# ofsoundof/NTIRE2022_ESR

Measured on AMD Instinct MI355X. Metric: images/sec (256x256->1024x1024 x4), higher is better.
Workload: dtype f32

## Files before the change

include/esr_hip.h:

```cpp
#ifndef ESR_HIP_H
#define ESR_HIP_H

#include <stddef.h>
#include <stdint.h>

#ifdef __cplusplus
extern "C" {
#endif

#define ESR_ABI_VERSION 12

typedef enum esr_status {
    ESR_OK = 0,
    ESR_ERR_BAD_ARG = -1,
    ESR_ERR_UNSUPPORTED = -2,
    ESR_ERR_LAUNCH = -3,
    ESR_ERR_TOO_SMALL = -4
} esr_status;

typedef enum esr_act { ESR_ACT_NONE = 0, ESR_ACT_LRELU = 1, ESR_ACT_RELU = 2, ESR_ACT_GELU = 3 } esr_act;

typedef enum esr_res { ESR_RES_NONE = 0, ESR_RES_PRE_ACT = 1, ESR_RES_POST_ACT = 2, ESR_RES_GATE = 3 } esr_res;

typedef enum esr_compute { ESR_COMPUTE_F32 = 0, ESR_COMPUTE_BF16 = 1, ESR_COMPUTE_F16 = 2 } esr_compute;
// ... 63 lines not shown
int    esr_pack_tail_s16(const float* w, const float* bias, int nseg, int seg_c, int mid_c, int cout, int compute, void* out, size_t out_bytes);
int    esr_conv_tail_supported(const esr_conv_desc* d);
int    esr_pack_conv_f32(const float* w_oihw, const float* bias, int cin, int cout, int ksize,
                         const int32_t* cin_map, int cin_phys, void* out, size_t out_bytes);
int    esr_unpack_conv_f32(const void* packed, size_t bytes, int cin, int cout, int ksize,
                           const int32_t* cin_map, int cin_phys, float* w_oihw, float* bias);

size_t esr_packed_conv_s16_bytes(int cin_phys, int cout, int ksize);
int    esr_pack_conv_s16(const float* w_oihw, const float* bias, int cin, int cout, int ksize, const int32_t* cin_map,
                         int cin_phys, int compute, void* out, size_t out_bytes);
int    esr_unpack_conv_s16(const void* packed, size_t bytes, int cin, int cout, int ksize, const int32_t* cin_map,
                           int cin_phys, int compute, float* w_oihw, float* bias);

size_t esr_packed_post_s16_bytes(int cin, int cout);
int    esr_pack_post_s16(const float* w_oi, const float* bias, int cin, int cout, int compute, void* out, size_t out_bytes);
int    esr_conv_post_supported(const esr_conv_desc* d);

size_t esr_packed_wino_bytes(int cin_phys, int cout);
int    esr_pack_wino_f32(const float* w_oihw, const float* bias, int cin, int cout, const int32_t* cin_map, int cin_phys,
                         void* out, size_t out_bytes);
int    esr_unpack_wino_f32(const void* packed, size_t bytes, int cin, int cout, const int32_t* cin_map, int cin_phys,
                           float* u_oc16, float* bias);
int    esr_wino_supported(const esr_conv_desc* d);

int esr_conv2d_f32(const esr_conv_desc* d, void* hip_stream);
int esr_conv_block_waves(const esr_conv_desc* d);

#define ESR_ESA_FP 16

size_t esr_packed_dense_bytes(int cin_p, int cout_p, int ksize);
int    esr_pack_dense_f32(const float* w_oihw, const float* bias, int cin, int cout, int ksize,
                          int cin_p, int cout_p, void* out, size_t out_bytes);

typedef struct esr_esa_post {
    int32_t cout;
    int32_t act;
    float   slope;
    int32_t res_mode;
    esr_view res;
    esr_view out;
} esr_esa_post;
int    esr_esa_apply_post_supported(int c, int cout0, int cout1);
size_t esr_packed_apply_post_bytes(int cin, int cout0, int cout1, int storage);
int    esr_pack_apply_post(const float* w0, const float* b0, const float* w1, const float* b1, int cin, int cout0, int cout1,
                           int storage, void* out, size_t out_bytes);

// ... 213 lines not shown
```

ntire2022_esr_amd/_lib.py:

```python
import ctypes
import os

_HERE = os.path.dirname(os.path.abspath(__file__))
SO_PATH = os.environ.get("ESR_HIP_LIB") or os.path.join(_HERE, "libesr_hip.so")

ESR_OK = 0
STATUS = {0: "ESR_OK", -1: "ESR_ERR_BAD_ARG", -2: "ESR_ERR_UNSUPPORTED", -3: "ESR_ERR_LAUNCH", -4: "ESR_ERR_TOO_SMALL"}

ACT_NONE, ACT_LRELU, ACT_RELU, ACT_GELU = 0, 1, 2, 3
RES_NONE, RES_PRE_ACT, RES_POST_ACT, RES_GATE = 0, 1, 2, 3
NHWC, NCHW_IN, NCHW_SHUFFLE4 = 0, 1, 2
BLOCKED_IN, BLOCKED_OUT1, BLOCKED_OUT0, BLOCKED_RES = 1, 2, 4, 8
HILO_IN, HILO_RES, HILO_OUT = 1, 2, 4
OP_CONV, OP_CONV3X3S2, OP_MAXPOOL7S3, OP_ESA_APPLY, OP_DWCONV, OP_BSCONV, OP_PACK_INPUT, OP_ESA_LOWRES, OP_CONV_CHAIN = 0, 1, 2, 3, 4, 5, 6, 7, 8
OP_MAXPOOL7S7 = 9
OP_DISTILL_STEP = 10
OP_RESBLOCK_HEAD = 11
OP_REFINE_CASCADE = 12
OP_DWCONV7 = 13
OP_CX_BLOCK = 14
OP_DWPW_PAIR = 15
OP_ESA_UNSHUFFLE = 16
OP_PA_GATE = 17
OP_PA_TAIL = 18
# ... 88 lines not shown
class ChainDesc(ctypes.Structure):
    _fields_ = [
        ("n", ctypes.c_int32), ("h", ctypes.c_int32), ("w", ctypes.c_int32), ("n_layers", ctypes.c_int32),
        ("cin", ctypes.c_int32), ("cmid", ctypes.c_int32), ("cout", ctypes.c_int32),
        ("act", ctypes.c_int32), ("slope", ctypes.c_float), ("res_mode", ctypes.c_int32),
        ("storage", ctypes.c_int32), ("compute", ctypes.c_int32),
        ("inp", View), ("wpacked", ctypes.c_void_p * CHAIN_MAX_LAYERS),
        ("post_wpacked", ctypes.c_void_p), ("post_out", View), ("post_cout", ctypes.c_int32), ("post_act", ctypes.c_int32),
        ("post2_wpacked", ctypes.c_void_p), ("post2_out", View), ("post2_cout", ctypes.c_int32), ("reserved", ctypes.c_int32),
    ]


class Op(ctypes.Structure):
    _fields_ = [("kind", ctypes.c_int32), ("reserved", ctypes.c_int32), ("conv", ConvDesc), ("esa", EsaDesc),
                ("bs", BsDesc), ("lo", EsaLowresDesc), ("chain", ChainDesc)]


EXPORTS = [
    "esr_abi_version", "esr_last_hip_error", "esr_build_info", "esr_source_hash", "esr_sizeof",
    "esr_packed_conv_bytes", "esr_pack_conv_f32", "esr_unpack_conv_f32",
    "esr_packed_conv_s16_bytes", "esr_pack_conv_s16", "esr_unpack_conv_s16",
    "esr_packed_post_s16_bytes", "esr_pack_post_s16", "esr_conv_post_supported",
    "esr_packed_tail_s16_bytes", "esr_pack_tail_s16", "esr_conv_tail_supported",
    "esr_packed_wino_bytes", "esr_pack_wino_f32", "esr_unpack_wino_f32", "esr_wino_supported",
    "esr_conv2d_f32", "esr_conv_block_waves", "esr_run_ops", "esr_pack_input_s16",
    "esr_prof_create", "esr_run_ops_profiled", "esr_prof_collect", "esr_prof_destroy", "esr_prof_kernel_symbol",
    "esr_packed_dense_bytes", "esr_pack_dense_f32",
    "esr_conv3x3s2_f32", "esr_maxpool7s3_f32", "esr_maxpool7s7_f32", "esr_esa_apply_f32", "esr_esa_lowres_f32",
    "esr_esa_apply_post_supported", "esr_packed_apply_post_bytes", "esr_pack_apply_post",
    "esr_packed_dw_bytes", "esr_pack_dw_f32", "esr_dwconv3x3_f32", "esr_bsconv_f32",
    "esr_tensor2uint_u8", "esr_sqerr_u8", "esr_channel_attention_f32",
    "esr_tensor2uint_u8_chk", "esr_ssim_partials", "esr_ssim_u8",
    "esr_conv_chain_supported", "esr_conv_chain_s16", "esr_distill_step_supported", "esr_distill_step_s16",
    "esr_resblock_head_supported", "esr_resblock_head_s16", "esr_refine_cascade_supported", "esr_refine_cascade_s16",
    "esr_packed_dw7_bytes", "esr_pack_dw7_f32", "esr_dwconv7x7_supported", "esr_dwconv7x7",
    "esr_packed_cx_pw1_bytes", "esr_pack_cx_pw1_s16", "esr_packed_cx_pw2_bytes", "esr_pack_cx_pw2_s16", "esr_cx_block_supported", "esr_cx_block_s16",
    "esr_dwpw_pair_supported", "esr_dwpw_pair_s16", "esr_esa_unshuffle_f32",
    "esr_packed_pa_gate_bytes", "esr_pack_pa_gate", "esr_pa_gate_supported", "esr_pa_gate", "esr_pa_tail_supported", "esr_pa_tail",
    "esr_packed_asym_s16_bytes", "esr_pack_asym_s16", "esr_unpack_asym_s16", "esr_asym_step_supported", "esr_asym_step",
    "esr_graph_create", "esr_graph_launch", "esr_graph_nodes", "esr_graph_destroy",
    "esr_event_pair_ms", "esr_bw_probe",
]

_lib = None


class EsrError(RuntimeError):
# ... 24 lines not shown
    L.esr_pack_conv_s16.restype = ci
    L.esr_unpack_conv_s16.argtypes = [vp, sz, ci, ci, ci, vp, ci, ci, vp, vp]
    L.esr_unpack_conv_s16.restype = ci
    L.esr_packed_post_s16_bytes.argtypes = [ci, ci]
    L.esr_packed_post_s16_bytes.restype = sz
    L.esr_pack_post_s16.argtypes = [vp, vp, ci, ci, ci, vp, sz]
    L.esr_pack_post_s16.restype = ci
    L.esr_packed_tail_s16_bytes.argtypes = [ci, ci, ci, ci]
    L.esr_packed_tail_s16_bytes.restype = sz
    L.esr_pack_tail_s16.argtypes = [vp, vp, ci, ci, ci, ci, ci, vp, sz]
    L.esr_pack_tail_s16.restype = ci
    L.esr_conv_tail_supported.argtypes = [ctypes.POINTER(ConvDesc)]
    L.esr_conv_tail_supported.restype = ci
    L.esr_conv_post_supported.argtypes = [ctypes.POINTER(ConvDesc)]
    L.esr_conv_post_supported.restype = ci
    L.esr_packed_wino_bytes.argtypes = [ci, ci]
    L.esr_packed_wino_bytes.restype = sz
    L.esr_pack_wino_f32.argtypes = [vp, vp, ci, ci, vp, ci, vp, sz]
    L.esr_pack_wino_f32.restype = ci
    L.esr_unpack_wino_f32.argtypes = [vp, sz, ci, ci, vp, ci, vp, vp]
    L.esr_unpack_wino_f32.restype = ci
    L.esr_wino_supported.argtypes = [ctypes.POINTER(ConvDesc)]
    L.esr_wino_supported.restype = ci
    L.esr_conv2d_f32.argtypes = [ctypes.POINTER(ConvDesc), vp]
    L.esr_conv2d_f32.restype = ci
    L.esr_conv_block_waves.argtypes = [ctypes.POINTER(ConvDesc)]
    L.esr_conv_block_waves.restype = ci
    L.esr_run_ops.argtypes = [ctypes.POINTER(Op), ci, vp]
    L.esr_run_ops.restype = ci
    L.esr_packed_dense_bytes.argtypes = [ci, ci, ci]
    L.esr_packed_dense_bytes.restype = sz
    L.esr_pack_dense_f32.argtypes = [vp, vp, ci, ci, ci, ci, ci, vp, sz]
    L.esr_pack_dense_f32.restype = ci
    for fn in (L.esr_conv3x3s2_f32, L.esr_maxpool7s3_f32, L.esr_maxpool7s7_f32, L.esr_esa_apply_f32):
        fn.argtypes = [ctypes.POINTER(EsaDesc), vp]
        fn.restype = ci
    L.esr_esa_lowres_f32.argtypes = [ctypes.POINTER(EsaLowresDesc), vp]
    L.esr_esa_lowres_f32.restype = ci
    L.esr_packed_dw_bytes.argtypes = [ci]
    L.esr_packed_dw_bytes.restype = sz
    L.esr_pack_dw_f32.argtypes = [vp, vp, ci, vp, sz]
    L.esr_pack_dw_f32.restype = ci
    L.esr_dwconv3x3_f32.argtypes = [ctypes.POINTER(ConvDesc), vp]
    L.esr_dwconv3x3_f32.restype = ci
    L.esr_bsconv_f32.argtypes = [ctypes.POINTER(BsDesc), vp]
    L.esr_bsconv_f32.restype = ci
# ... 121 lines not shown
```

ntire2022_esr_amd/csrc/esr_hip.hip:

```cpp
#include <hip/hip_runtime.h>
#include <stddef.h>
#include <math.h>
#include <stdarg.h>
#include <stdint.h>
#include <stdio.h>
#include <string.h>
#include <stdlib.h>
#include <type_traits>

#include "esr_hip.h"
#include "esr_internal.h"

typedef float f32x4 __attribute__((ext_vector_type(4)));
typedef float f32x2 __attribute__((ext_vector_type(2)));

namespace {

constexpr int TILE = 16;
constexpr int CHUNK = 8;
constexpr int THREADS = 256;

struct ConvK {
    const float* x;
    const float* wp;
// ... 6 lines not shown
    int cin;
    int in_pitch, in_coff;
    int res_pitch, res_coff;
    int y0_pitch, y0_coff, y1_pitch, y1_coff;
    int cout_store;
    int split;
    int act;
    float slope;
    int res_mode;
    int out_layout;
    int tiles_x, tiles_y;
    const float* wp2;
    const float* bias2;
    const float* cat;
    int cat_pitch, cat_coff, cat_chunks;
    int mid_act;
    const float* wp3; const float* bias3; float* y2;
    int y2_pitch, y2_coff, y2_cout4, post_act, post_nch8;
    int res_in;
    int out16;
    int y1_blk;
    int in_blk;
    int y0_blk, res_blk;
};

__device__ __forceinline__ float act_any(float v, int act, float slope)
{
    switch (act) {
        case ESR_ACT_LRELU: return fmaxf(v, slope * v);
        case ESR_ACT_RELU: return fmaxf(v, 0.f);
        case ESR_ACT_GELU: return 0.5f * v * (1.f + erff(v * 0.70710678118654752440f));
        default: return v;
    }
}

template <int ACT>
__device__ __forceinline__ f32x4 act4(f32x4 v, float slope)
{
    if (ACT == ESR_ACT_LRELU) {
        const f32x4 m = v * slope;
        v.x = fmaxf(v.x, m.x); v.y = fmaxf(v.y, m.y); v.z = fmaxf(v.z, m.z); v.w = fmaxf(v.w, m.w);
    } else if (ACT == ESR_ACT_RELU) {
        v.x = fmaxf(v.x, 0.f); v.y = fmaxf(v.y, 0.f); v.z = fmaxf(v.z, 0.f); v.w = fmaxf(v.w, 0.f);
    } else if (ACT == ESR_ACT_GELU) {
        v.x = 0.5f * v.x * (1.f + erff(v.x * 0.70710678118654752440f));
        v.y = 0.5f * v.y * (1.f + erff(v.y * 0.70710678118654752440f));
// ... 219 lines not shown
    for (int r = 0; r < 4; ++r) {
        const int gy = y0 + wv * 4 + r;
        if (gy >= p.H) continue;
#pragma unroll
        for (int t = 0; t < NT; ++t) {
            if (t * 16 + kq * 4 >= p.cout_store) continue;
            f32x4 v = acc[t][r];
            if (p.act != ESR_ACT_NONE || p.res_mode != ESR_RES_NONE) {
                f32x4 rvv = {0.f, 0.f, 0.f, 0.f};
                if (p.res_mode != ESR_RES_NONE) {
                    const int pix = (n * p.H + gy) * p.W + gx;
                    rvv = *reinterpret_cast<const f32x4*>(p.res + (size_t)(pix * p.res_pitch + p.res_coff + t * 16 + kq * 4));
                }
                if (p.res_mode == ESR_RES_PRE_ACT) v += rvv;
                v.x = act_any(v.x, p.act, p.slope); v.y = act_any(v.y, p.act, p.slope);
                v.z = act_any(v.z, p.act, p.slope); v.w = act_any(v.w, p.act, p.slope);
                if (p.res_mode == ESR_RES_POST_ACT) v += rvv;
            }
            float* dst = p.y0 + (((size_t)n * nco + t) * H4 + (size_t)gy * 4 + kq) * W4 + (size_t)gx * 4;
            *reinterpret_cast<f32x4*>(dst) = v;
        }
    }
}

constexpr int TAIL_C16 = 4;

template <int NT, int KS, bool IN_NCHW, int NW, int TNT = 0, int PNT = 0, bool Y1BLK = false>
__global__ __launch_bounds__(64 * NW, 2) void conv_f32_kernel(const ConvK p)
{
    static_assert(!Y1BLK || (NT == 4 && KS == 3 && !IN_NCHW && TNT == 0 && PNT == 0), "blocked y1: the 64-output 3x3 with a split store");
    static_assert(PNT == 0 || (TNT == 0 && KS == 3 && !IN_NCHW && NW == 8), "post 1x1: 8-wave 3x3 NHWC kernels");
    static_assert(TNT == 0 || (NT == 1 && KS == 3 && !IN_NCHW && NW == 4), "tail: 3x3, <= 16 channels, 4-wave blocks");
    constexpr int THREADS = 64 * NW;
    constexpr int TILE_H = 4 * NW;
    constexpr int HALO = KS / 2;
    constexpr int TH = TILE + 2 * HALO;
    constexpr int THY = TILE_H + 2 * HALO;
    constexpr int NPX = TH * THY;
    constexpr int TAPS = KS * KS;
    constexpr int IN_ITEMS = 2 * NPX;
    constexpr int IN_BYTES = IN_ITEMS * 16;
    constexpr int W_ITEMS = TAPS * NT * 32;
    constexpr int W_FLOATS = W_ITEMS * 4;
    constexpr int STAGE_BYTES = IN_BYTES + W_ITEMS * 16;
    constexpr int IN_ROUNDS = (IN_ITEMS + THREADS - 1) / THREADS;
    constexpr int W_ROUNDS = (W_ITEMS + THREADS - 1) / THREADS;
    constexpr unsigned OOB = 0x80000000u;

    constexpr int TAIL_FLOATS = TNT ? TAIL_C16 * TNT * 256 + TNT * 16 : (PNT ? NT * PNT * 256 + PNT * 16 : 0);
    __shared__ __attribute__((aligned(16))) char smem[2 * STAGE_BYTES + NW * EPI_WAVE_FLOATS * 4 + TAIL_FLOATS * 4];

    __builtin_amdgcn_s_setprio(3);

    const int tid = threadIdx.x;
    const int lane = tid & 63;
    const int wv = tid >> 6;
    const int px = lane & 15;
    const int kq = lane >> 4;
    float* const scr = reinterpret_cast<float*>(smem + 2 * STAGE_BYTES) + wv * EPI_WAVE_FLOATS;

    const int ntiles = p.N * p.tiles_y * p.tiles_x;
    const int G = gridDim.x;
    auto tile_index = [&](int k) -> int {
        const int base = k * G;
        if (base >= ntiles) return -1;
        int off = blockIdx.x;
        if ((G & 7) == 0 && base + G <= ntiles) off = (blockIdx.x & 7) * (G >> 3) + (blockIdx.x >> 3);
        const int t = base + off;
        return t < ntiles ? t : -1;
    };

    struct TileCtx { int n, x0, y0; unsigned voff[IN_ROUNDS]; };
    auto setup_tile = [&](int t, TileCtx& c) {
        const int tx = t % p.tiles_x;
// ... 294 lines not shown
                        v.x = act_any(v.x, p.post_act, p.slope); v.y = act_any(v.y, p.post_act, p.slope);
                        v.z = act_any(v.z, p.post_act, p.slope); v.w = act_any(v.w, p.post_act, p.slope);
                        *reinterpret_cast<f32x4*>(dst + td * 16 + kq * 4) = v;
                    }
                }
            }
            epilogue_nhwc<NT>(p, acc, scr, cur.n, cur.x0, cur.y0, wv, lane, TILE_H);
        } else if (p.out_layout == ESR_NCHW_SHUFFLE4) epilogue_shuffle<NT>(p, acc, cur.n, cur.x0, cur.y0, wv, lane);
        else if (IN_NCHW && p.out16) epilogue_nhwc_store16<NT>(p, acc, cur.n, cur.x0, cur.y0, wv, lane);
        else epilogue_nhwc<NT, Y1BLK>(p, acc, scr, cur.n, cur.x0, cur.y0, wv, lane, TILE_H);
        if (!has_next) break;
        cur = nxt;
        ++k;
        tn = tile_index(k + 1);
        if (tn >= 0) setup_tile(tn, nxt);
    }
}

#include "imdb_tail.inc"

thread_local char g_err[256] = "";
thread_local char g_kname[256] = "";
thread_local bool g_ktrace = false;

constexpr int TALL_MIN_TILES = 256;
inline int conv_block_waves(int ksize, bool in_nchw, int nt, int nchunks, int n, int h, int w)
{
    const int tall_min = TALL_MIN_TILES;
    if (ksize != 3 || in_nchw || nt < 3 || nchunks < 2) return 4;
    const long ntall = (long)n * ((w + TILE - 1) / TILE) * ((h + 31) / 32);
    return ntall >= tall_min ? 8 : 4;
}

template <int NT, int KS, bool IN_NCHW>
int launch_conv(const ConvK& k, hipStream_t st)
{
    const int ntiles = k.N * k.tiles_x * k.tiles_y;
    constexpr bool CAN_TALL = KS == 3 && !IN_NCHW && NT >= 3;
    if (CAN_TALL && conv_block_waves(KS, IN_NCHW, NT, k.nchunks, k.N, k.H, k.W) == 8) {
        const int tall_y = (k.H + 31) / 32;
        const int ntall = k.N * k.tiles_x * tall_y;
        ConvK kk = k;
        kk.tiles_y = tall_y;
        const int grid = esr_persistent_grid(ntall, ESR_BLOCKS_1_PER_CU);
        esr_note_kernel("conv_f32_kernel<%d, %d, %s, 8, 0, %d, %s>", NT, KS, esr_tf(IN_NCHW), (NT == 4 && kk.wp3) ? 2 : 0, esr_tf(NT == 4 && !kk.wp3 && kk.y1_blk));
        if (NT == 4 && kk.wp3)
            hipLaunchKernelGGL((conv_f32_kernel<NT, KS, IN_NCHW, CAN_TALL ? 8 : 4, 0, (CAN_TALL && NT == 4) ? 2 : 0>), dim3(grid), dim3(512), 0, st, kk);
        else if (NT == 4 && kk.y1_blk)
            hipLaunchKernelGGL((conv_f32_kernel<NT, KS, IN_NCHW, CAN_TALL ? 8 : 4, 0, 0, CAN_TALL && NT == 4>), dim3(grid), dim3(512), 0, st, kk);
        else
            hipLaunchKernelGGL((conv_f32_kernel<NT, KS, IN_NCHW, CAN_TALL ? 8 : 4>), dim3(grid), dim3(512), 0, st, kk);
        esr_graph_note_io(st, kk.x, offsetof(ConvK, x), kk.y0, offsetof(ConvK, y0));
        return esr_check_launch("conv_f32_kernel (tall) launch");
    }
    const int grid = esr_persistent_grid(ntiles, ESR_BLOCKS_2_PER_CU);
    esr_note_kernel("conv_f32_kernel<%d, %d, %s, 4, 0, 0, %s>", NT, KS, esr_tf(IN_NCHW), esr_tf(CAN_TALL && NT == 4 && k.y1_blk));
    if (CAN_TALL && NT == 4 && k.y1_blk) hipLaunchKernelGGL((conv_f32_kernel<NT, KS, IN_NCHW, 4, 0, 0, CAN_TALL && NT == 4>), dim3(grid), dim3(THREADS), 0, st, k);
    else hipLaunchKernelGGL((conv_f32_kernel<NT, KS, IN_NCHW, 4>), dim3(grid), dim3(THREADS), 0, st, k);
    esr_graph_note_io(st, k.x, offsetof(ConvK, x), k.y0, offsetof(ConvK, y0));
    return esr_check_launch("conv_f32_kernel launch");
}

inline bool imdb_tail_shape(const ConvK& k)
{
    if (k.nchunks != IT_NCH || k.cat_chunks != IT_CAT || k.cout_store != 64) return false;
    if (k.res_mode != ESR_RES_NONE && k.res_mode != ESR_RES_PRE_ACT) return false;
    const double px = (double)k.H * k.W;
    return esr_fits_raw(px, k.in_pitch, 4) && esr_fits_raw(px, k.cat_pitch, 4) && (k.res_mode == ESR_RES_NONE || esr_fits_raw(px, k.res_pitch, 4));
}

int launch_conv_tail(const ConvK& k, hipStream_t st)
{
    const int ntiles = k.N * k.tiles_x * k.tiles_y;
    const int grid = esr_persistent_grid(ntiles, ESR_BLOCKS_2_PER_CU);
    if (imdb_tail_shape(k)) {
        ConvK kk = k;
        kk.res_mode = ESR_RES_NONE;
        kk.tiles_y = (k.H + 4 * IT_NW - 1) / (4 * IT_NW);
// ... 132 lines not shown
int esr_unpack_conv_f32(const void* packed, size_t bytes, int cin, int cout, int ksize,
                        const int32_t* cin_map, int cin_phys, float* w, float* bias)
{
    if (!packed || !w || cin <= 0 || cout <= 0 || (ksize != 1 && ksize != 3)) return ESR_ERR_BAD_ARG;
    if (bytes < esr_packed_conv_bytes(cin_phys, cout, ksize)) return ESR_ERR_BAD_ARG;
    const int nt = esr_round_up(cout, 16) / 16, taps = ksize * ksize;
    const float* o = static_cast<const float*>(packed);
    memset(w, 0, sizeof(float) * (size_t)cout * cin * taps);
    for (int s = 0; s < cin_phys; ++s) {
        const int c = cin_map ? cin_map[s] : (s < cin ? s : -1);
        if (c < 0) continue;
        for (int oc = 0; oc < cout; ++oc)
            for (int tap = 0; tap < taps; ++tap) {
                int j;
                w[((size_t)oc * cin + c) * taps + tap] = o[pack_index(nt, taps, s, tap, oc, &j)];
            }
    }
    if (bias) {
        const float* bo = o + (size_t)(esr_round_up(cin_phys, CHUNK) / CHUNK) * taps * nt * 128;
        for (int oc = 0; oc < cout; ++oc) bias[oc] = bo[oc];
    }
    return ESR_OK;
}

int esr_conv_block_waves(const esr_conv_desc* d)
{
    if (!d || d->cin <= 0 || d->cout <= 0) return 0;
    if (d->storage != ESR_STORE_F32 && d->in_layout == ESR_NHWC) return esr_s16_block_waves(d);
    const bool in_nchw = d->in_layout == ESR_NCHW_IN;
    const int cin_phys = in_nchw ? CHUNK : esr_round_up(d->cin, CHUNK);
    return conv_block_waves(d->ksize, in_nchw, esr_round_up(d->cout, 16) / 16, cin_phys / CHUNK, d->n, d->h, d->w);
}

int esr_conv2d_f32(const esr_conv_desc* d, void* hip_stream)
{
    if (!d || !d->in.ptr || !d->wpacked) return ESR_ERR_BAD_ARG;
    if (!d->out0.ptr && !(d->post_wpacked && d->storage != ESR_STORE_F32)) return ESR_ERR_BAD_ARG;
    if (d->n <= 0 || d->h <= 0 || d->w <= 0 || d->cin <= 0 || d->cout <= 0) return ESR_ERR_BAD_ARG;
    if (d->ksize != 1 && d->ksize != 3) return ESR_ERR_UNSUPPORTED;
    if (d->cout > 64) return ESR_ERR_UNSUPPORTED;
    const bool in_nchw = d->in_layout == ESR_NCHW_IN;
    if (in_nchw && (d->cin > 4 || d->ksize != 3)) return ESR_ERR_UNSUPPORTED;
    if (!in_nchw && d->in_layout != ESR_NHWC) return ESR_ERR_BAD_ARG;
    const bool store16 = d->storage == ESR_STORE_BF16 || d->storage == ESR_STORE_F16;
    if (d->storage != ESR_STORE_F32 && !store16) return ESR_ERR_BAD_ARG;
    if (d->res_mode == ESR_RES_GATE && (d->act != ESR_ACT_NONE || d->out_layout != ESR_NHWC || d->tail_wpacked || d->post_wpacked || d->hilo))
// ... 33 lines not shown
    int split = d->split <= 0 ? cout4 : d->split;
    if (split >= ecout) split = cout4;
    if (split & 3) return ESR_ERR_BAD_ARG;
    if (d->out_layout == ESR_NCHW_SHUFFLE4) {
        if (ecout % 16) return ESR_ERR_UNSUPPORTED;
    } else if (d->out_layout == ESR_NHWC) {
        if (!esr_view_fits(d->out0, 4, split)) return ESR_ERR_BAD_ARG;
        if (split < cout4 && !esr_view_ok(d->out1, 4, cout4 - split)) return ESR_ERR_BAD_ARG;
    } else {
        return ESR_ERR_BAD_ARG;
    }
    if (d->res_mode != ESR_RES_NONE && !esr_view_ok(d->res, 4, cout4)) return ESR_ERR_BAD_ARG;
    {
        const double px_all = (double)d->n * d->h * d->w, px_img = (double)d->h * d->w;
        int maxpitch = in_nchw ? 4 : d->in.pitch;
        if (d->out_layout == ESR_NHWC) maxpitch = maxpitch > d->out0.pitch ? maxpitch : d->out0.pitch;
        if (d->out_layout == ESR_NHWC && d->out1.ptr) maxpitch = maxpitch > d->out1.pitch ? maxpitch : d->out1.pitch;
        if (d->res_mode != ESR_RES_NONE) maxpitch = maxpitch > d->res.pitch ? maxpitch : d->res.pitch;
        if (!esr_fits_raw(px_all, maxpitch, 1)) return ESR_ERR_UNSUPPORTED;
        if (!esr_fits_raw(px_img, in_nchw ? d->cin : d->in.pitch, 4)) return ESR_ERR_UNSUPPORTED;
    }

    if (d->blocked8 & ~(ESR_BLOCKED_IN | ESR_BLOCKED_OUT1 | ESR_BLOCKED_OUT0 | ESR_BLOCKED_RES)) return ESR_ERR_BAD_ARG;
    if ((d->blocked8 & (ESR_BLOCKED_OUT0 | ESR_BLOCKED_RES)) && (!tail || store16)) return ESR_ERR_UNSUPPORTED;
    if (d->wino_wpacked && !store16 && esr_wino_supported(d)) return esr_conv2d_wino(d, hip_stream);

    const int nt = esr_round_up(d->cout, 16) / 16;
    const int taps = d->ksize * d->ksize;
    ConvK k;
    k.out16 = store16 ? d->storage : 0;
    k.x = static_cast<const float*>(d->in.ptr);
    k.wp = static_cast<const float*>(d->wpacked);
    k.nchunks = cin_phys / CHUNK;
    k.bias = k.wp + (size_t)k.nchunks * taps * nt * 128;
    k.res = static_cast<const float*>(d->res.ptr);
    k.y0 = static_cast<float*>(d->out0.ptr);
    k.y1 = static_cast<float*>(d->out1.ptr);
    k.N = d->n; k.H = d->h; k.W = d->w;
    k.cin = d->cin;
    k.in_pitch = d->in.pitch; k.in_coff = d->in.coff;
    k.res_pitch = d->res.pitch; k.res_coff = d->res.coff;
    k.y0_pitch = d->out0.pitch; k.y0_coff = d->out0.coff;
    k.y1_pitch = d->out1.pitch; k.y1_coff = d->out1.coff;
    k.cout_store = cout4;
    k.split = split;
    k.act = d->act; k.slope = d->slope; k.res_mode = d->res_mode;
    k.res_in = 0;
    k.y1_blk = (d->blocked8 & ESR_BLOCKED_OUT1) ? 1 : 0;
    k.in_blk = (d->blocked8 & ESR_BLOCKED_IN) ? 1 : 0;
    k.y0_blk = (d->blocked8 & ESR_BLOCKED_OUT0) ? 1 : 0;
    k.res_blk = (d->blocked8 & ESR_BLOCKED_RES) ? 1 : 0;
    const double px = (double)d->h * d->w;
    if (k.y0_blk && (!esr_view_aligned(d->out0, 8) || !esr_fits_raw(px, d->out0.pitch, 4))) return ESR_ERR_UNSUPPORTED;
    if (k.res_blk && (d->res_mode != ESR_RES_PRE_ACT || !esr_view_aligned(d->res, 8))) return ESR_ERR_UNSUPPORTED;
    if (k.y1_blk) {
        if (d->out_layout != ESR_NHWC || tail || post || store16 || split >= cout4 || d->ksize != 3 || in_nchw || d->cout <= 48 || d->cout > 64 || !esr_view_aligned(d->out1, 8) || (split & 7) ||
            !esr_fits_raw(px, d->out1.pitch, 4))
            return ESR_ERR_UNSUPPORTED;
    }
    if (k.in_blk && (!tail || in_nchw || !esr_view_aligned(d->in, 8))) return ESR_ERR_UNSUPPORTED;
    if (!tail && d->ksize == 3 && !in_nchw && esr_res_is_input(d, 1)) {
        k.res_in = 1;
        k.res_mode = ESR_RES_NONE;
    }
    k.out_layout = d->out_layout;
    k.tiles_x = (d->w + TILE - 1) / TILE;
    k.tiles_y = (d->h + TILE - 1) / TILE;
    k.wp2 = nullptr; k.bias2 = nullptr; k.cat = nullptr; k.cat_pitch = k.cat_coff = k.cat_chunks = 0; k.mid_act = ESR_ACT_NONE;
    k.wp3 = nullptr; k.bias3 = nullptr; k.y2 = nullptr; k.y2_pitch = k.y2_coff = k.y2_cout4 = 0; k.post_act = ESR_ACT_NONE; k.post_nch8 = 0;
    if (post) {
        if (conv_block_waves(3, false, nt, k.nchunks, d->n, d->h, d->w) != 8) {
            esr_conv_desc a = *d;
            a.post_wpacked = nullptr;
            const int rc = esr_conv2d_f32(&a, hip_stream);
// ... 160 lines not shown
```

ntire2022_esr_amd/engine.py:

```python
import collections
import ctypes
import itertools
import threading
import types
import weakref
from dataclasses import dataclass

import numpy as np
import torch
import torch.nn as nn

from . import _lib as L


def _ptr(t):
    return None if t is None else ctypes.c_void_p(t.data_ptr())


def _host(t):
    return None if t is None else t.detach().to("cpu", torch.float32).contiguous()


def _pack_args(weight=None, bias=None, cin=None, cin_map=None, cin_phys=None, compute=None, flat=False):
    w = _host(weight)
# ... 556 lines not shown
                if not L.lib().esr_conv_tail_supported(ctypes.byref(d)):
                    raise L.EsrError(f"{self.w}: no fused tail kernel for this shape (the plan should have built separate ops)")
            elif psfx and not L.lib().esr_conv_post_supported(ctypes.byref(d)):
                raise L.EsrError(f"{self.w}: no fused post-chain kernel for this shape (the plan should have built separate ops)")

    def cost(self, plan, desc):
        es = plan.esize
        hw = self.hw
        npix = plan.npix if hw is None else plan.n * hw[0] * hw[1]
        e_act = es if hw is None else 4
        nt = (self.cout + 15) // 16
        nw = L.lib().esr_conv_block_waves(ctypes.byref(desc.conv)) if desc is not None else 0
        kern = f"conv_f32_kernel<NT={nt},KS={self.k},NCHW_IN={int(self.src is INPUT)},NW={nw}>"
        if self.s16(plan):
            kern = f"conv_s16_kernel<NT={nt},KS={self.k},NW={nw or 8},{plan.store}>"
        blk = isinstance(self.dst1, Buffer) and self.dst1.blocked
        if blk:
            kern = kern[:-1] + ",BLK>"
        wino = desc is not None and bool(desc.conv.wino_wpacked) and bool(L.lib().esr_wino_supported(ctypes.byref(desc.conv)))
        if wino:
            rm = self.res_mode if self.res is not None else L.RES_NONE
            at = self.act if (self.act == L.ACT_LRELU or (self.act == L.ACT_NONE and rm != L.RES_POST_ACT)) else -1
            kern = f"wino_f32_kernel<{at}, {rm}, {2 if self.dst is OUTPUT else int(blk)}>"
        e_in = 4 if self.src is INPUT else e_act
        e_out = 4 if self.dst is OUTPUT else e_act
        ca, co, k = self.cin_alg, self.cout, self.k
        res_read = self.res is not None and not _same_view(self.res, self.src)
        wb = 4.0 * ca * co * k ** 2
        rd = npix * (ca * e_in + (co * e_act if res_read else 0)) + wb
        if self.head:
            rd += npix * (16 * 2 - ca * e_in)
        wr = float(npix * co * e_out) if self.dst is not None else 0.0
        hl = self.hilo
        rd += npix * e_act * ((ca if hl & L.HILO_IN else 0) + (co if (hl & L.HILO_RES and res_read) else 0))
        wr += npix * e_act * co if hl & L.HILO_OUT else 0.0
        if hl:
            kern = kern[:-1] + ",HILO>"
        flops = 2.0 * npix * ca * co * k * k
        if self.bs_of is not None:
            flops = 2.0 * npix * (ca * co + 9 * co)
            wb = 4.0 * (ca * co + 10 * co)
            rd = npix * (ca * e_in + (co * e_act if res_read else 0)) + wb
            if self.head:
                rd += npix * (16 * 2 - ca * e_in)
        tl = self.tail
        if tl is not None:
# ... 18 lines not shown
                kern = kern[:-1] + f"+{(pt.post2.cout + 15) // 16}>"
                flops += 2.0 * npix * pt.cout * pt.post2.cout
                wr += npix * e_act * pt.post2.cout
        chunk = 8 if es == 4 else 16
        hl_in, hl_res, hl_out = (2 if hl & L.HILO_IN else 1), (2 if hl & L.HILO_RES else 1), (2 if hl & L.HILO_OUT else 1)
        sc = lambda v, logical: _stored_channels(v.seg(0) if (isinstance(v, Planar) and hl) else v, logical, chunk)
        st = 16 * 2 * npix if self.head else npix * e_in * hl_in * sc(self.src, ca)
        if tl is not None:
            st += npix * e_act * sc(tl.cat, tl.cat_c)
        if res_read:
            st += npix * e_act * hl_res * sc(self.res, co if tl is None else tl.cout)
        if self.dst is not None:
            st += npix * e_out * hl_out * sc(self.dst, self.split if self.dst1 is not None else (co if tl is None else tl.cout))
        if self.dst1 is not None:
            st += npix * e_act * sc(self.dst1, co - self.split)
        if pt is not None:
            st += npix * e_act * sc(pt.dst, pt.cout)
            if pt.post2 is not None:
                st += npix * e_act * sc(pt.post2.dst, pt.post2.cout)
            wb += 4.0 * co * pt.cout + (4.0 * pt.cout * pt.post2.cout if pt.post2 is not None else 0.0)
        fexec = flops * (16.0 / 36.0) if wino else flops
        if hl & L.HILO_IN:
            fexec = 2.0 * flops
        return _cost(self.w, kern, self.cin, co, k, flops, rd, wr, float(st) + wb, fexec)

    def counted_convs(self, plan):
        if not self.counted:
            return []
        npix = plan.npix if self.hw is None else plan.n * self.hw[0] * self.hw[1]
        conv = (self.cin_alg, self.cout, self.k, npix, self.act)
        t = self.tail
        if t is not None:
            return [conv[:4] + (t.mid_act,), (t.cat_c + self.cout, t.cout, 1, npix, self.act)]
        t = self.post
        if t is not None:
            r = [conv, (self.cout, t.cout, 1, npix, t.act)]
            if t.post2 is not None:
                r.append((t.cout, t.post2.cout, 1, npix, L.ACT_NONE))
            return r
        return [conv]


@dataclass
class Dw(_Op):
    w: str
    src: object
# ... 1338 lines not shown
```

ntire2022_esr_amd/ops.py:

```python
import contextlib
import ctypes

import torch

from . import _lib as L
from .engine import (pack_asym_s16, pack_conv, pack_conv_s16, pack_cx_pw, pack_distill_s16, pack_dw, pack_dw7, pack_dwpw_pw, pack_pa_gate, pack_post_s16,
                     pack_unshuffle, pack_wino)


def _view(t, coff=0):
    return L.View(ctypes.c_void_p(t.data_ptr()), t.shape[-1], coff)


_STORE_OF = {torch.float32: "f32", torch.bfloat16: "bf16", torch.float16: "f16"}


def _provided(t, what, like, shape, cmin, gran):
    if not isinstance(t, torch.Tensor) or t.device != like.device:
        raise L.EsrError(f"{what}: must be a tensor on {like.device}")
    if t.dtype != like.dtype:
        raise L.EsrError(f"{what}: dtype {t.dtype}, the op stores {like.dtype}")
    if not t.is_contiguous() or tuple(t.shape[:-1]) != tuple(shape):
        raise L.EsrError(f"{what}: must be a contiguous [{', '.join(str(v) for v in shape)}, pitch] tensor, got {tuple(t.shape)}")
    if t.shape[-1] % gran or t.shape[-1] < cmin:
# ... 34 lines not shown
    if _TRACE is None or kind is None:
        L.check(getattr(lib, fn)(ctypes.byref(d), ctypes.c_void_p(stream)), what)
        return
    op = L.Op()
    op.kind = kind
    setattr(op, field, d)
    prof = ctypes.c_void_p()
    L.check(lib.esr_prof_create(1, 1, ctypes.byref(prof)), "esr_prof_create")
    try:
        L.check(lib.esr_run_ops_profiled(ctypes.byref(op), 1, ctypes.c_void_p(stream), prof), what)
        buf = ctypes.create_string_buffer(256)
        L.check(lib.esr_prof_kernel_symbol(prof, 0, buf, 256), "esr_prof_kernel_symbol")
        _TRACE.append(buf.value.decode())
    finally:
        (torch.cuda.ExternalStream(stream) if stream else torch.cuda.default_stream()).synchronize()
        lib.esr_prof_destroy(prof)


def conv2d(x, weight, bias, *, act=L.ACT_NONE, slope=0.05, res=None, res_mode=L.RES_NONE,
           in_nchw=False, shuffle_out=False, out=None, out_coff=0, in_coff=0, cin=None,
           split=0, out1=None, out1_coff=0, res_coff=0, packed=None, cin_map=None, store=None,
           tail_weight=None, tail_bias=None, tail_cat=None, tail_cat_coff=0, tail_mid_act=L.ACT_NONE,
           post_weight=None, post_bias=None, post_act=L.ACT_NONE, post2_weight=None, post2_bias=None, store_main=True,
           border=None, blocked_in=False, blocked_out1=False, wino=False, hilo=0, post_out=None, post2_out=None):
    if not x.is_cuda:
        raise L.EsrError("conv2d: tensors must live on the GPU; there is no CPU fallback")
    lib = L.lib()
    w4 = weight if weight.dim() == 4 else weight[:, :, None, None]
    cout, wcin, k, _ = w4.shape
    st = _STORE_OF[x.dtype] if not in_nchw else (store or "f32")
    s16 = st != "f32" and not in_nchw
    if packed is None:
        packed = (pack_conv_s16(weight, bias, st, cin_map=cin_map) if s16 else pack_conv(weight, bias, cin_map=cin_map)).to(x.device)
    odt = {"f32": torch.float32, "bf16": torch.bfloat16, "f16": torch.float16}[st]
    gran = 4 if st == "f32" else 8
    d = L.ConvDesc()
    d.storage = L.STORE[st]
    d.compute = L.COMPUTE[st] if s16 else 0
    hilo_strides = []
    if in_nchw:
        n, c, h, w = x.shape
        d.in_layout, cin = L.NCHW_IN, c
        d.inp = L.View(ctypes.c_void_p(x.data_ptr()), 0, 0)
    elif blocked_in:
        if x.dim() != 5 or x.shape[-1] != 8 or x.dtype != torch.float32 or not x.is_contiguous():
            raise L.EsrError("conv2d: a blocked input is a contiguous fp32 [N, C/8, H, W, 8] tensor")
        n, pl, h, w, _ = x.shape
# ... 24 lines not shown
        d.inp = _view(x, in_coff)
    d.n, d.h, d.w, d.cin, d.cout, d.ksize = n, h, w, cin, cout, k
    keep = None
    if tail_weight is not None:
        tw = tail_weight if tail_weight.dim() == 4 else tail_weight[:, :, None, None]
        keep = pack_conv(tw, tail_bias).to(x.device)
        d.tail_wpacked = ctypes.c_void_p(keep.data_ptr())
        d.tail_cat = _view(tail_cat, tail_cat_coff)
        d.tail_cat_c, d.tail_cout, d.tail_mid_act = tw.shape[1] - 16, tw.shape[0], tail_mid_act
        cout = tw.shape[0]
    d.act, d.slope, d.res_mode, d.split = act, slope, res_mode, split
    if border is not None:
        if border.dtype != torch.float32 or not border.is_contiguous() or tuple(border.shape) != (16, (cout + 15) // 16 * 16):
            raise L.EsrError("conv2d: border must be a contiguous fp32 [16, round_up(cout, 16)] tensor")
        d.border_bias = ctypes.c_void_p(border.data_ptr())
    if shuffle_out:
        y = torch.empty((n, cout // 16, 4 * h, 4 * w), dtype=torch.float32, device=x.device) if out is None else out
        d.out_layout = L.NCHW_SHUFFLE4
        d.out0 = L.View(ctypes.c_void_p(y.data_ptr()), 0, 0)
    else:
        d.out_layout = L.NHWC
        if not store_main:
            y = None
        else:
            if out is None:
                c_store = (min(split, cout) if split else cout)
                y = torch.zeros(((2,) if hilo & L.HILO_OUT else ()) + (n, h, w, (c_store + gran - 1) // gran * gran if not hilo & L.HILO_OUT else (cout + 15) // 16 * 16),
                                dtype=odt, device=x.device)
            else:
                y = out
            if hilo & L.HILO_OUT:
                if y.dim() != 5 or y.shape[0] != 2 or not y.is_contiguous():
                    raise L.EsrError("conv2d: a hi + lo output is a contiguous [2, N, H, W, P] pair")
                d.out0 = _view(y[0], out_coff)
                _hilo_pair(y, "output", hilo_strides)
            else:
                d.out0 = _view(y, out_coff)
        if out1 is not None:
            if blocked_out1:
                if out1.dim() != 5 or out1.shape[-1] != 8 or out1.dtype != torch.float32 or not out1.is_contiguous():
                    raise L.EsrError("conv2d: a blocked out1 is a contiguous fp32 [N, C/8, H, W, 8] tensor")
                d.out1 = L.View(ctypes.c_void_p(out1.data_ptr()), out1.shape[1] * 8, out1_coff)
                d.blocked8 |= L.BLOCKED_OUT1
            else:
                d.out1 = _view(out1, out1_coff)
    if res is not None and hilo & L.HILO_RES:
# ... 653 lines not shown
```

Before: 1770.

## Add MFMA-based head conv kernel for NCHW low-channel 3x3 input convolution

Adds a specialized path for the first 3x3 convolution, which reads NCHW input with at most 4 input channels. Each wave handles a 16-pixel-wide strip and slides a 3-row window of buffer loads down the band. It computes all output channels with f32 MFMA instructions, applies bias and leaky ReLU, and stages the result through LDS. The result is stored to NHWC or 8-channel blocked layout using 128-bit buffer stores. The path replaces the generic tiled conv kernel for this layer, which wastes work on the tiny input channel count. It adds a new blocked-output option and a persistent grid of a quarter as many blocks, and is enabled by default through a global mode flag.

New measurement: 1779, median of 6. No clear change (+0.5%).

```diff
diff --git a/include/esr_hip.h b/include/esr_hip.h
--- a/include/esr_hip.h
+++ b/include/esr_hip.h
@@ -109,6 +109,7 @@
 int    esr_unpack_wino_f32(const void* packed, size_t bytes, int cin, int cout, const int32_t* cin_map, int cin_phys,
                            float* u_oc16, float* bias);
 int    esr_wino_supported(const esr_conv_desc* d);
+int    esr_head_supported(const esr_conv_desc* d);
 
 int esr_conv2d_f32(const esr_conv_desc* d, void* hip_stream);
 int esr_conv_block_waves(const esr_conv_desc* d);
diff --git a/ntire2022_esr_amd/_lib.py b/ntire2022_esr_amd/_lib.py
--- a/ntire2022_esr_amd/_lib.py
+++ b/ntire2022_esr_amd/_lib.py
@@ -134,7 +134,7 @@
     "esr_packed_conv_s16_bytes", "esr_pack_conv_s16", "esr_unpack_conv_s16",
     "esr_packed_post_s16_bytes", "esr_pack_post_s16", "esr_conv_post_supported",
     "esr_packed_tail_s16_bytes", "esr_pack_tail_s16", "esr_conv_tail_supported",
-    "esr_packed_wino_bytes", "esr_pack_wino_f32", "esr_unpack_wino_f32", "esr_wino_supported",
+    "esr_packed_wino_bytes", "esr_pack_wino_f32", "esr_unpack_wino_f32", "esr_wino_supported", "esr_head_supported",
     "esr_conv2d_f32", "esr_conv_block_waves", "esr_run_ops", "esr_pack_input_s16",
     "esr_prof_create", "esr_run_ops_profiled", "esr_prof_collect", "esr_prof_destroy", "esr_prof_kernel_symbol",
     "esr_packed_dense_bytes", "esr_pack_dense_f32",
@@ -205,6 +205,8 @@
     L.esr_unpack_wino_f32.restype = ci
     L.esr_wino_supported.argtypes = [ctypes.POINTER(ConvDesc)]
     L.esr_wino_supported.restype = ci
+    L.esr_head_supported.argtypes = [ctypes.POINTER(ConvDesc)]
+    L.esr_head_supported.restype = ci
     L.esr_conv2d_f32.argtypes = [ctypes.POINTER(ConvDesc), vp]
     L.esr_conv2d_f32.restype = ci
     L.esr_conv_block_waves.argtypes = [ctypes.POINTER(ConvDesc)]
diff --git a/ntire2022_esr_amd/csrc/esr_head.inc b/ntire2022_esr_amd/csrc/esr_head.inc
--- /dev/null
+++ b/ntire2022_esr_amd/csrc/esr_head.inc
@@ -0,0 +1,116 @@
+typedef int i32x4 __attribute__((ext_vector_type(4)));
+
+constexpr int HD_NW = 4;
+constexpr int HD_ROWS = 16;
+constexpr int HD_PITCH = 68;
+constexpr unsigned HD_OOB = 0x80000000u;
+constexpr int HD_RSRC = 0x00020000;
+
+template <int NT, bool BLK>
+__device__ __forceinline__ void head_f32_body(const ConvK& p, float* smem)
+{
+    const int lane = threadIdx.x & 63;
+    const int wv = __builtin_amdgcn_readfirstlane(threadIdx.x >> 6);
+    const int px = lane & 15, kq = lane >> 4;
+    float* const scr = smem + wv * (16 * HD_PITCH);
+
+    const int ch = ((kq & 1) << 1) | (kq >> 1);
+    float wr[9][NT];
+#pragma unroll
+    for (int tap = 0; tap < 9; ++tap)
+#pragma unroll
+        for (int t = 0; t < NT; ++t) wr[tap][t] = p.wp[((tap * NT + t) * 64 + (ch >> 1) * 16 + px) * 2 + (ch & 1)];
+    f32x4 biasv[NT];
+#pragma unroll
+    for (int t = 0; t < NT; ++t) biasv[t] = *reinterpret_cast<const f32x4*>(p.bias + t * 16 + kq * 4);
+
+    const float slope = p.act == ESR_ACT_LRELU ? p.slope : 1.f;
+    const int plane = p.H * p.W;
+    const int img_bytes = p.cin * plane * 4;
+    const int nitems = p.N * p.tiles_y * p.tiles_x;
+    const int ngroups = (nitems + HD_NW - 1) / HD_NW;
+    const int G = gridDim.x;
+    const int c4 = lane & 15, hf = lane & 1, pp = lane >> 5;
+    const int sp = BLK ? (lane >> 1) & 15 : lane >> 4;
+    constexpr int NST = BLK ? NT : 4;
+
+    for (int k = 0;; ++k) {
+        const int base = k * G;
+        if (base >= ngroups) break;
+        int off = blockIdx.x;
+        if ((G & 7) == 0 && base + G <= ngroups) off = (blockIdx.x & 7) * (G >> 3) + (blockIdx.x >> 3);
+        const int item = (base + off) * HD_NW + wv;
+        if (item >= nitems) continue;
+        const int tx = item % p.tiles_x;
+        const int q = item / p.tiles_x;
+        const int band = q % p.tiles_y;
+        const int n = q / p.tiles_y;
+        const int x0 = tx * 16, yb = band * HD_ROWS;
+        const int rows = min(HD_ROWS, p.H - yb);
+
+        const float* const ximg = p.x + (size_t)n * p.cin * plane;
+        unsigned coff[3];
+#pragma unroll
+        for (int d = 0; d < 3; ++d) {
+            const int gx = x0 + px + d - 1;
+            coff[d] = (ch < p.cin && gx >= 0 && gx < p.W) ? (unsigned)(ch * plane + gx) * 4u : HD_OOB;
+        }
+        auto load_row = [&](int gy, float (&v)[3]) {
+            const __amdgpu_buffer_rsrc_t xr = __builtin_amdgcn_make_buffer_rsrc(const_cast<float*>(ximg), 0, (gy >= 0 && gy < p.H) ? img_bytes : 0, HD_RSRC);
+            const unsigned ro = (unsigned)(gy * p.W) * 4u;
+#pragma unroll
+            for (int d = 0; d < 3; ++d) v[d] = __builtin_bit_cast(float, __builtin_amdgcn_raw_buffer_load_b32(xr, coff[d] + ro, 0, 0));
+        };
+        unsigned soff[NST];
+#pragma unroll
+        for (int i = 0; i < NST; ++i) {
+            const int gx = x0 + (BLK ? sp : sp + 4 * i);
+            if (BLK) soff[i] = gx < p.W ? ((unsigned)((2 * i + pp) * plane + gx) * 8u + 4u * hf) * 4u : HD_OOB;
+            else soff[i] = (gx < p.W && c4 * 4 < NT * 16) ? (unsigned)(gx * p.y0_pitch + c4 * 4) * 4u : HD_OOB;
+        }
+        float* const y0 = BLK ? p.y0 + ((size_t)n * (p.y0_pitch >> 3) + (p.y0_coff >> 3)) * plane * 8
+                              : p.y0 + (size_t)n * plane * p.y0_pitch + p.y0_coff;
+        const int ybytes = BLK ? ((p.y0_pitch - p.y0_coff) >> 3) * plane * 32 : (p.W * p.y0_pitch - p.y0_coff) * 4;
+
+        float in[3][3];
+        load_row(yb - 1, in[0]);
+        load_row(yb, in[1]);
+        load_row(yb + 1, in[2]);
+
+        for (int r = 0; r < rows; ++r) {
+            const int gy = yb + r;
+            float nx[3];
+            load_row(gy + 2, nx);
+            __builtin_amdgcn_sched_barrier(0);
+
+            f32x4 acc[NT];
+#pragma unroll
+            for (int t = 0; t < NT; ++t) acc[t] = biasv[t];
+#pragma unroll
+            for (int tap = 0; tap < 9; ++tap)
+#pragma unroll
+                for (int t = 0; t < NT; ++t)
+                    acc[t] = __builtin_amdgcn_mfma_f32_16x16x4f32(wr[tap][t], in[tap / 3][tap % 3], acc[t], 0, 0, 0);
+
+#pragma unroll
+            for (int t = 0; t < NT; ++t) {
+                f32x4 v = acc[t];
+                const f32x4 m = v * slope;
+                v.x = fmaxf(v.x, m.x); v.y = fmaxf(v.y, m.y); v.z = fmaxf(v.z, m.z); v.w = fmaxf(v.w, m.w);
+                *reinterpret_cast<f32x4*>(scr + px * HD_PITCH + t * 16 + kq * 4) = v;
+            }
+            const size_t row_floats = BLK ? (size_t)gy * p.W * 8 : (size_t)gy * p.W * p.y0_pitch;
+            const __amdgpu_buffer_rsrc_t yr = __builtin_amdgcn_make_buffer_rsrc(y0 + row_floats, 0, BLK ? ybytes - gy * p.W * 32 : ybytes, HD_RSRC);
+            f32x4 o[NST];
+#pragma unroll
+            for (int i = 0; i < NST; ++i) {
+                const int fl = BLK ? sp * HD_PITCH + (2 * i + pp) * 8 + 4 * hf : (sp + 4 * i) * HD_PITCH + (NT == 4 ? c4 * 4 : min(c4 * 4, NT * 16 - 4));
+                o[i] = *reinterpret_cast<const f32x4*>(scr + fl);
+            }
+#pragma unroll
+            for (int i = 0; i < NST; ++i) __builtin_amdgcn_raw_buffer_store_b128(__builtin_bit_cast(i32x4, o[i]), yr, soff[i], 0, 0);
+#pragma unroll
+            for (int d = 0; d < 3; ++d) { in[0][d] = in[1][d]; in[1][d] = in[2][d]; in[2][d] = nx[d]; }
+        }
+    }
+}
diff --git a/ntire2022_esr_amd/csrc/esr_hip.hip b/ntire2022_esr_amd/csrc/esr_hip.hip
--- a/ntire2022_esr_amd/csrc/esr_hip.hip
+++ b/ntire2022_esr_amd/csrc/esr_hip.hip
@@ -52,6 +52,7 @@
     int y1_blk;
     int in_blk;
     int y0_blk, res_blk;
+    int head;
 };
 
 __device__ __forceinline__ float act_any(float v, int act, float slope)
@@ -317,6 +318,8 @@
         }
     }
 }
+
+#include "esr_head.inc"
 
 constexpr int TAIL_C16 = 4;
 
@@ -345,6 +348,13 @@
     constexpr int TAIL_FLOATS = TNT ? TAIL_C16 * TNT * 256 + TNT * 16 : (PNT ? NT * PNT * 256 + PNT * 16 : 0);
     __shared__ __attribute__((aligned(16))) char smem[2 * STAGE_BYTES + NW * EPI_WAVE_FLOATS * 4 + TAIL_FLOATS * 4];
 
+    if constexpr (IN_NCHW) {
+        if (p.head) {
+            if (p.y0_blk) head_f32_body<NT, true>(p, reinterpret_cast<float*>(smem));
+            else head_f32_body<NT, false>(p, reinterpret_cast<float*>(smem));
+            return;
+        }
+    }
     __builtin_amdgcn_s_setprio(3);
 
     const int tid = threadIdx.x;
@@ -685,6 +695,7 @@
 thread_local char g_err[256] = "";
 thread_local char g_kname[256] = "";
 thread_local bool g_ktrace = false;
+int g_head_mode = 1;
 
 constexpr int TALL_MIN_TILES = 256;
 inline int conv_block_waves(int ksize, bool in_nchw, int nt, int nchunks, int n, int h, int w)
@@ -716,7 +727,7 @@
         esr_graph_note_io(st, kk.x, offsetof(ConvK, x), kk.y0, offsetof(ConvK, y0));
         return esr_check_launch("conv_f32_kernel (tall) launch");
     }
-    const int grid = esr_persistent_grid(ntiles, ESR_BLOCKS_2_PER_CU);
+    const int grid = esr_persistent_grid((IN_NCHW && k.head) ? (ntiles + 3) / 4 : ntiles, ESR_BLOCKS_2_PER_CU);
     esr_note_kernel("conv_f32_kernel<%d, %d, %s, 4, 0, 0, %s>", NT, KS, esr_tf(IN_NCHW), esr_tf(CAN_TALL && NT == 4 && k.y1_blk));
     if (CAN_TALL && NT == 4 && k.y1_blk) hipLaunchKernelGGL((conv_f32_kernel<NT, KS, IN_NCHW, 4, 0, 0, CAN_TALL && NT == 4>), dim3(grid), dim3(THREADS), 0, st, k);
     else hipLaunchKernelGGL((conv_f32_kernel<NT, KS, IN_NCHW, 4>), dim3(grid), dim3(THREADS), 0, st, k);
@@ -895,6 +906,23 @@
     }
     return ESR_OK;
 }
+
+int esr_head_supported(const esr_conv_desc* d)
+{
+    if (!d) return 0;
+    if (d->in_layout != ESR_NCHW_IN || d->ksize != 3 || d->cin < 1 || d->cin > 4) return 0;
+    if (d->storage != ESR_STORE_F32 || d->compute != ESR_COMPUTE_F32) return 0;
+    if (d->cout < 16 || d->cout > 64 || (d->cout & 15)) return 0;
+    if (d->res_mode != ESR_RES_NONE || d->tail_wpacked || d->post_wpacked || d->post2_wpacked || d->hilo || d->border_bias || d->in_seg_stride) return 0;
+    if (d->split > 0 && d->split < d->cout) return 0;
+    if (d->act != ESR_ACT_NONE && d->act != ESR_ACT_LRELU) return 0;
+    if (d->out_layout != ESR_NHWC) return 0;
+    if (d->blocked8 & ~ESR_BLOCKED_OUT0) return 0;
+    if ((d->blocked8 & ESR_BLOCKED_OUT0) && !esr_view_aligned(d->out0, 8)) return 0;
+    return 1;
+}
+
+void esr_dbg_head(int on) { g_head_mode = on ? 1 : 0; }
 
 int esr_conv_block_waves(const esr_conv_desc* d)
 {
@@ -974,7 +1002,8 @@
     }
 
     if (d->blocked8 & ~(ESR_BLOCKED_IN | ESR_BLOCKED_OUT1 | ESR_BLOCKED_OUT0 | ESR_BLOCKED_RES)) return ESR_ERR_BAD_ARG;
-    if ((d->blocked8 & (ESR_BLOCKED_OUT0 | ESR_BLOCKED_RES)) && (!tail || store16)) return ESR_ERR_UNSUPPORTED;
+    const bool head = g_head_mode && esr_head_supported(d);
+    if ((d->blocked8 & (ESR_BLOCKED_OUT0 | ESR_BLOCKED_RES)) && !head && (!tail || store16)) return ESR_ERR_UNSUPPORTED;
     if (d->wino_wpacked && !store16 && esr_wino_supported(d)) return esr_conv2d_wino(d, hip_stream);
 
     const int nt = esr_round_up(d->cout, 16) / 16;
@@ -1002,6 +1031,8 @@
     k.in_blk = (d->blocked8 & ESR_BLOCKED_IN) ? 1 : 0;
     k.y0_blk = (d->blocked8 & ESR_BLOCKED_OUT0) ? 1 : 0;
     k.res_blk = (d->blocked8 & ESR_BLOCKED_RES) ? 1 : 0;
+    k.head = head ? 1 : 0;
+    if (head && !esr_fits_raw((double)d->w, d->out0.pitch, 4)) return ESR_ERR_UNSUPPORTED;
     const double px = (double)d->h * d->w;
     if (k.y0_blk && (!esr_view_aligned(d->out0, 8) || !esr_fits_raw(px, d->out0.pitch, 4))) return ESR_ERR_UNSUPPORTED;
     if (k.res_blk && (d->res_mode != ESR_RES_PRE_ACT || !esr_view_aligned(d->res, 8))) return ESR_ERR_UNSUPPORTED;
diff --git a/ntire2022_esr_amd/engine.py b/ntire2022_esr_amd/engine.py
--- a/ntire2022_esr_amd/engine.py
+++ b/ntire2022_esr_amd/engine.py
@@ -602,6 +602,7 @@
             rm = self.res_mode if self.res is not None else L.RES_NONE
             at = self.act if (self.act == L.ACT_LRELU or (self.act == L.ACT_NONE and rm != L.RES_POST_ACT)) else -1
             kern = f"wino_f32_kernel<{at}, {rm}, {2 if self.dst is OUTPUT else int(blk)}>"
+        head = desc is not None and bool(L.lib().esr_head_supported(ctypes.byref(desc.conv)))
         e_in = 4 if self.src is INPUT else e_act
         e_out = 4 if self.dst is OUTPUT else e_act
         ca, co, k = self.cin_alg, self.cout, self.k
@@ -666,6 +667,8 @@
         fexec = flops * (16.0 / 36.0) if wino else flops
         if hl & L.HILO_IN:
             fexec = 2.0 * flops
+        if head:
+            fexec = 2.0 * npix * 4 * (16 * nt) * 9
         return _cost(self.w, kern, self.cin, co, k, flops, rd, wr, float(st) + wb, fexec)
 
     def counted_convs(self, plan):
diff --git a/ntire2022_esr_amd/ops.py b/ntire2022_esr_amd/ops.py
--- a/ntire2022_esr_amd/ops.py
+++ b/ntire2022_esr_amd/ops.py
@@ -80,7 +80,7 @@
            split=0, out1=None, out1_coff=0, res_coff=0, packed=None, cin_map=None, store=None,
            tail_weight=None, tail_bias=None, tail_cat=None, tail_cat_coff=0, tail_mid_act=L.ACT_NONE,
            post_weight=None, post_bias=None, post_act=L.ACT_NONE, post2_weight=None, post2_bias=None, store_main=True,
-           border=None, blocked_in=False, blocked_out1=False, wino=False, hilo=0, post_out=None, post2_out=None):
+           border=None, blocked_in=False, blocked_out1=False, blocked_out0=False, wino=False, hilo=0, post_out=None, post2_out=None):
     if not x.is_cuda:
         raise L.EsrError("conv2d: tensors must live on the GPU; there is no CPU fallback")
     lib = L.lib()
@@ -151,6 +151,13 @@
         d.out_layout = L.NHWC
         if not store_main:
             y = None
+        elif blocked_out0:
+            if out is None or out.dim() != 5 or out.shape[-1] != 8 or out.dtype != torch.float32 or not out.is_contiguous() or \
+                    tuple(out.shape[2:4]) != (h, w) or out.shape[0] != n:
+                raise L.EsrError("conv2d: a blocked out is a caller-provided contiguous fp32 [N, C/8, H, W, 8] tensor")
+            y = out
+            d.out0 = L.View(ctypes.c_void_p(y.data_ptr()), y.shape[1] * 8, out_coff)
+            d.blocked8 |= L.BLOCKED_OUT0
         else:
             if out is None:
                 c_store = (min(split, cout) if split else cout)
```
